# leggedrobotics/art_planner

Measured on NVIDIA H100. Metric: pose-validity checks/s, higher is better.
Workload: dtype f32

## Files before the change

### art_planner_b200/csrc/artp_capi.cu

```cuda
#include <cassert>
#include <climits>
#include <cmath>
#include <cstdlib>
#include <cstring>
#include <type_traits>
#include <vector>

#include "artp_internal.h"
#include "artp_kernels.cuh"
#include "artp_tiles.cuh"

using namespace artp_api;

namespace {

thread_local std::string g_create_error;

__global__ void reverse_columns_kernel(const float* __restrict__ layer, float* __restrict__ H, int nx, int nz, int pitch) {
  const size_t total = (size_t)pitch * nz;
  for (size_t i = blockIdx.x * (size_t)blockDim.x + threadIdx.x; i < total; i += (size_t)gridDim.x * blockDim.x) {
    const int z = (int)(i / pitch), x = (int)(i - (size_t)z * pitch);
    H[i] = (x < nx) ? layer[x + (size_t)(nz - 1 - z) * nx] * 1.0f + 0.0f : 0.0f;
  }
}
// ... 62 lines not shown
  base = lo <= hi ? lo : 0.0f;
  int e = -126;
  while (e < 127 && artp::code_dec(base, std::ldexp(1.0f, e), artp::kCodeMax) < hi) ++e;
  step = std::ldexp(1.0f, e);
}

struct PlaneSlot { unsigned long long key; uint32_t lo, hi; };
constexpr unsigned long long kEmptyKey = ~0ull;
__device__ __forceinline__ unsigned long long plane_key(int kx, int kz, int kd) {
  return ((unsigned long long)(uint32_t)(kx & 0xffff) << 48) | ((unsigned long long)(uint32_t)(kz & 0xffff) << 32) | (uint32_t)kd;
}
__device__ __forceinline__ uint32_t plane_slot_hash(unsigned long long k) {
  k ^= k >> 33; k *= 0xff51afd7ed558ccdull; k ^= k >> 33; k *= 0xc4ceb9fe1a85ec53ull; k ^= k >> 33;
  return (uint32_t)k;
}
__global__ void plane_table_clear_kernel(PlaneSlot* tab, size_t cap) {
  for (size_t i = blockIdx.x * (size_t)blockDim.x + threadIdx.x; i < cap; i += (size_t)gridDim.x * blockDim.x) {
    tab[i].key = kEmptyKey; tab[i].lo = 0xffffffffu; tab[i].hi = 0u;
  }
}
__device__ __forceinline__ bool cell_tri_plane(const artp::Field& f, int x, int x_off, int z, int u, float pl[4]) {
  float hA, hB, hC, hD;
  artp::load_cell(f, x, z, hA, hB, hC, hD);
  const bool ok = u == 0 ? (artp::finitef(hA) && artp::finitef(hB) && artp::finitef(hC))
                         : (artp::finitef(hD) && artp::finitef(hB) && artp::finitef(hC));
  if (!ok) return false;
  artp::cell_plane(f, u == 0, x + x_off, z, hA, hB, hC, hD, pl);
  return true;
}
__global__ void plane_table_insert_kernel(const artp::Field f, int x_off, PlaneSlot* tab, uint32_t mask) {
  const size_t ncell = (size_t)(f.nx - 1) * (f.nz - 1);
  for (size_t i = blockIdx.x * (size_t)blockDim.x + threadIdx.x; i < 2 * ncell; i += (size_t)gridDim.x * blockDim.x) {
    const size_t c = i >> 1;
    const int u = (int)(i & 1), z = (int)(c / (f.nx - 1)), x = (int)(c - (size_t)z * (f.nx - 1));
    float pl[4];
    if (!cell_tri_plane(f, x, x_off, z, u, pl)) continue;
    const uint32_t id = (uint32_t)(((size_t)z * f.pitch + x) * 2 + u);
    const unsigned long long key = plane_key(artp::nkey(pl[0]), artp::nkey(pl[2]), artp::dkey(pl[3]));
    uint32_t s = plane_slot_hash(key) & mask;
    for (;;) {
      const unsigned long long old = atomicCAS(&tab[s].key, kEmptyKey, key);
      if (old == kEmptyKey || old == key) {
        if (!(tab[s].lo < id && tab[s].hi > id)) { atomicMin(&tab[s].lo, id); atomicMax(&tab[s].hi, id); }
        break;
      }
      s = (s + 1) & mask;
    }
  }
}
__global__ void plane_table_query_kernel(const artp::Field f, int x_off, const PlaneSlot* __restrict__ tab, uint32_t mask,
                                         unsigned char* __restrict__ mergeable) {
  const size_t ncell = (size_t)(f.nx - 1) * (f.nz - 1);
  for (size_t i = blockIdx.x * (size_t)blockDim.x + threadIdx.x; i < 2 * ncell; i += (size_t)gridDim.x * blockDim.x) {
    const size_t c = i >> 1;
    const int u = (int)(i & 1), z = (int)(c / (f.nx - 1)), x = (int)(c - (size_t)z * (f.nx - 1));
    float pl[4];
    if (!cell_tri_plane(f, x, x_off, z, u, pl)) continue;
    const uint32_t id = (uint32_t)(((size_t)z * f.pitch + x) * 2 + u);
    const float e2 = 2.0f * ARTP_EPS;
    const int kx0 = artp::nkey(pl[0] - e2), kx1 = artp::nkey(pl[0] + e2);
    const int kz0 = artp::nkey(pl[2] - e2), kz1 = artp::nkey(pl[2] + e2);
    const int kd0 = artp::dkey(pl[3] - e2), kd1 = artp::dkey(pl[3] + e2);
    bool dup = false;
    for (int kx = kx0; kx <= kx1 && !dup; ++kx)
      for (int kz = kz0; kz <= kz1 && !dup; ++kz)
        for (int kd = kd0; kd <= kd1 && !dup; ++kd) {
          const unsigned long long key = plane_key(kx, kz, kd);
          uint32_t s = plane_slot_hash(key) & mask;
          for (;;) {
            const unsigned long long k = tab[s].key;
            if (k == kEmptyKey) break;
            if (k == key) { dup = tab[s].lo != id || tab[s].hi != id; break; }
            s = (s + 1) & mask;
          }
        }
    if (dup) mergeable[(size_t)z * f.pitch + x] = 2;
  }
}

__global__ void fill_u8_kernel(uint8_t* p, size_t n, uint8_t v) {
  for (size_t i = blockIdx.x * (size_t)blockDim.x + threadIdx.x; i < n; i += (size_t)gridDim.x * blockDim.x) p[i] = v;
}

constexpr int kCompactBlock = 1024;
template <bool BITS>
__device__ __forceinline__ int mask_at(const uint8_t* __restrict__ valid, size_t i) {
  if (BITS) return (int)((reinterpret_cast<const uint32_t*>(valid)[i >> 5] >> (i & 31)) & 1u);
  return valid[i] != 0;
}
template <bool BITS>
__global__ void compact_count_kernel(const uint8_t* __restrict__ valid, size_t n, uint32_t* __restrict__ counts) {
  const size_t i = (size_t)blockIdx.x * kCompactBlock + threadIdx.x;
  const int v = (i < n) && mask_at<BITS>(valid, i);
  const int c = __syncthreads_count(v);
  if (threadIdx.x == 0) counts[blockIdx.x] = (uint32_t)c;
}
__global__ void compact_scan_kernel(uint32_t* counts, size_t nb, uint32_t* total) {
  __shared__ uint32_t carry;
  __shared__ uint32_t wsum[32];
  if (threadIdx.x == 0) carry = 0;
  __syncthreads();
  for (size_t b0 = 0; b0 < nb; b0 += blockDim.x) {
    const size_t i = b0 + threadIdx.x;
    const uint32_t v = i < nb ? counts[i] : 0u;
    uint32_t x = v;
    const int lane = threadIdx.x & 31, wid = threadIdx.x >> 5;
    for (int o = 1; o < 32; o <<= 1) { const uint32_t y = __shfl_up_sync(0xffffffffu, x, o); if (lane >= o) x += y; }
    if (lane == 31) wsum[wid] = x;
    __syncthreads();
    if (wid == 0) {
      uint32_t s = lane < (int)(blockDim.x >> 5) ? wsum[lane] : 0u;
      for (int o = 1; o < 32; o <<= 1) { const uint32_t y = __shfl_up_sync(0xffffffffu, s, o); if (lane >= o) s += y; }
      wsum[lane] = s;
    }
    __syncthreads();
    const uint32_t before = carry + (wid ? wsum[wid - 1] : 0u) + x - v;
    if (i < nb) counts[i] = before;
    __syncthreads();
    if (threadIdx.x == blockDim.x - 1) carry = before + v;
    __syncthreads();
  }
  if (threadIdx.x == 0) *total = carry;
}
template <bool BITS, typename IndexT>
__global__ void compact_scatter_kernel(const uint8_t* __restrict__ valid, size_t n, int64_t base,
                                       const uint32_t* __restrict__ offsets, IndexT* __restrict__ out) {
  __shared__ uint32_t wsum[32];
  const size_t i = (size_t)blockIdx.x * kCompactBlock + threadIdx.x;
  const int v = (i < n) && mask_at<BITS>(valid, i);
  const unsigned bal = __ballot_sync(0xffffffffu, v);
  const int lane = threadIdx.x & 31, wid = threadIdx.x >> 5;
  if (lane == 0) wsum[wid] = __popc(bal);
  __syncthreads();
  if (wid == 0) {
    uint32_t s = wsum[lane];
    for (int o = 1; o < 32; o <<= 1) { const uint32_t y = __shfl_up_sync(0xffffffffu, s, o); if (lane >= o) s += y; }
    wsum[lane] = s;
  }
  __syncthreads();
  if (v) {
    const uint32_t pos = offsets[blockIdx.x] + (wid ? wsum[wid - 1] : 0u) + __popc(bal & ((1u << lane) - 1u));
    out[pos] = (IndexT)(base + (int64_t)i);
  }
}

__global__ void pack_bits_kernel(const uint8_t* __restrict__ valid, size_t n, uint32_t* __restrict__ bits) {
  const size_t words = (n + 31) / 32;
  const size_t warps = ((size_t)gridDim.x * blockDim.x) >> 5, wid = ((size_t)blockIdx.x * blockDim.x + threadIdx.x) >> 5;
  const int lane = threadIdx.x & 31;
  for (size_t w = wid; w < words; w += warps) {
    const size_t i = w * 32 + lane;
    const unsigned bal = __ballot_sync(0xffffffffu, i < n && valid[i] != 0);
    if (lane == 0) bits[w] = bal;
  }
}

constexpr size_t kChunkItems = 1u << 20;

int ensure_queues(Handle* h, size_t n_items) {
  const size_t need = 5 * std::min(n_items, kChunkItems);
  if (h->recs_cap >= need) return ARTP_OK;
  const size_t cap = std::max<size_t>(need, 1u << 16);
  h->recs_cap = 0;
  size_t had[4] = {0, 0, 0, 0};
  int rc;
  TRY(grow(h, h->d_recs, had[0], cap));
  TRY(grow(h, h->d_recs_f, had[1], cap));
  TRY(grow(h, h->d_recs_g, had[2], cap));
  TRY(grow(h, h->d_defer, had[3], cap));
  h->recs_cap = cap;
  return ARTP_OK;
}

struct HostFeed {
  const char* host;
  char* dev;
  size_t bytes_per_item;
  size_t slice_items;
  float schedule[8];
};
constexpr size_t kScheduleItems = 1u << 18;
constexpr int kPipeReachCtasPerSm = 2;

__global__ void close_slice_kernel(const BoxQueues* round, BoxQueues* slices, int i) {
  const BoxQueues prev = i ? slices[i - 1] : BoxQueues{};
  slices[i].group = {round->group.end, prev.group.end};
  slices[i].reach = {round->reach.end, prev.reach.end};
  slices[i].big = {round->big.end, prev.big.end};
}

int launch_classify(Handle* h, artp::Work w, size_t lo, size_t hi, cudaStream_t s) {
  w.item_base = (uint32_t)lo;
  w.n_items = (uint32_t)hi;
  BoxQueues* q = &h->d_ctr->q;
  return launch(h, artp::classify_items_kernel, (unsigned)((hi - lo + artp::kClassifyItems - 1) / artp::kClassifyItems),
                artp::kClassifyItems, 0, s, h->chk, w, h->d_recs, h->d_recs_f, h->group_grid ? h->d_recs_g : nullptr, &q->big.end,
                &q->reach.end, &q->group.end, h->mode == 1);
}

int launch_big_tile(Handle* h, artp::Work w, size_t lo, size_t hi, BoxQueues* q, cudaStream_t s) {
  w.item_base = (uint32_t)lo;
  w.n_items = (uint32_t)hi;
  const int wpc = h->tile_warps[0];
  const unsigned grid = (unsigned)std::min<size_t>((size_t)h->tile_grid[0], (5 * (hi - lo) + wpc - 1) / wpc);
  return launch(h, artp::box_tiles_warp_kernel, grid, wpc * 32, h->tile_smem[0], s, h->chk, h->tile_map[0][0], h->tile_map[0][1],
                h->tile_cfg[0], w, h->d_recs, &q->big.end, &q->big.claim, &h->d_ctr->defer, h->d_defer, 0u, h->mode == 1);
}
int launch_reach_warp(Handle* h, artp::Work w, size_t lo, size_t hi, BoxQueues* q, cudaStream_t s, unsigned reach_cap) {
  if (!h->chk.reach_tw) return ARTP_OK;
  w.item_base = (uint32_t)lo;
  w.n_items = (uint32_t)hi;
  const int wpc = h->tile_warps[1];
  const unsigned grid = (unsigned)std::min<size_t>({(size_t)h->tile_grid[1], (4 * (hi - lo) + wpc - 1) / wpc, reach_cap});
  return launch(h, artp::box_tiles_warp_kernel, grid, wpc * 32, h->tile_smem[1], s, h->chk, h->tile_map[1][1], h->tile_map[1][1],
                h->tile_cfg[1], w, h->d_recs_f, &q->reach.end, &q->reach.claim, &h->d_ctr->defer, h->d_defer, artp::kDeferReachBit,
                h->mode == 1);
}
int launch_reach_groups(Handle* h, artp::Work w, size_t lo, size_t hi, BoxQueues* q, cudaStream_t s, unsigned reach_cap) {
  if (!h->group_grid) return ARTP_OK;
  w.item_base = (uint32_t)lo;
  w.n_items = (uint32_t)hi;
  const unsigned grid = (unsigned)std::min<size_t>({(size_t)h->group_grid, (hi - lo + 7) / 8, reach_cap});
  return launch(h, artp::reach_groups_kernel, grid, artp::kMaxTileWarps * 32, h->group_smem, s, h->chk, h->tile_map[1][1],
                h->tile_cfg[1], w, h->d_recs_g, &q->group.end, &q->group.claim);
}

int launch_grouping(Handle* h, artp::Work w, size_t lo, size_t hi, cudaStream_t s) {
  w.item_base = (uint32_t)lo;
  w.n_items = (uint32_t)hi;
  const unsigned grid = (unsigned)std::min<size_t>((size_t)h->k2_grid, 5 * (hi - lo));
  return launch(h, artp::box_items_block_kernel, grid, artp::kBlockStageThreads, h->k2_smem, s, h->chk, w, h->d_recs, h->d_recs_f,
                &h->d_ctr->defer, h->d_defer, h->k2_tcap, h->d_err);
}

int run_round_device(Handle* h, const artp::Work& w, cudaStream_t s, size_t base, size_t end, bool timed) {
  CU_TRY(h, cudaMemsetAsync(h->d_ctr, 0, sizeof(Counters), s));
  if (timed) CU_TRY(h, cudaEventRecord(h->ev[0], s));
  TRY(launch_classify(h, w, base, end, s));
  if (timed) CU_TRY(h, cudaEventRecord(h->ev[1], s));
  const bool fork = !h->timing && h->chk.reach_tw;
  if (fork) {
    CU_TRY(h, cudaEventRecord(h->slice_ev[0], s));
    CU_TRY(h, cudaStreamWaitEvent(h->box_stream, h->slice_ev[0], 0));
    if (h->group_grid) CU_TRY(h, cudaStreamWaitEvent(h->group_stream, h->slice_ev[0], 0));
  }
  BoxQueues* q = &h->d_ctr->q;
  TRY(launch_big_tile(h, w, base, end, q, s));
  if (timed) CU_TRY(h, cudaEventRecord(h->ev[2], s));
  TRY(launch_reach_warp(h, w, base, end, q, fork ? h->box_stream : s, UINT_MAX));
  if (timed) CU_TRY(h, cudaEventRecord(h->ev[3], s));
  TRY(launch_reach_groups(h, w, base, end, q, fork ? h->group_stream : s, UINT_MAX));
  if (fork) {
    CU_TRY(h, cudaEventRecord(h->box_ev, h->box_stream));
    CU_TRY(h, cudaStreamWaitEvent(s, h->box_ev, 0));
    if (h->group_grid) {
      CU_TRY(h, cudaEventRecord(h->group_ev, h->group_stream));
      CU_TRY(h, cudaStreamWaitEvent(s, h->group_ev, 0));
    }
  }
  if (timed) CU_TRY(h, cudaEventRecord(h->ev[4], s));
  TRY(launch_grouping(h, w, base, end, s));
  if (timed) { CU_TRY(h, cudaEventRecord(h->ev[5], s)); h->ev_valid = true; }
  return ARTP_OK;
}

int run_round_piped(Handle* h, const artp::Work& w, cudaStream_t s, const HostFeed& feed, size_t base, size_t end) {
  size_t cut[kMaxSlices + 1];
  int ncut = 0;
  cut[0] = base;
  if (end - base >= kScheduleItems) {
    double acc = 0.0;
    for (int i = 0; i < 8 && feed.schedule[i] > 0.0f; ++i) {
      acc += feed.schedule[i];
      const size_t c = std::min(end, (base + (size_t)((double)(end - base) * acc) + 127) & ~(size_t)127);
      if (c > cut[ncut]) cut[++ncut] = c;
    }
    if (cut[ncut] != end) cut[++ncut] = end;
  } else {
    for (size_t lo = base; lo < end; lo += feed.slice_items) cut[++ncut] = std::min(end, lo + feed.slice_items);
  }
  assert(ncut <= kMaxSlices);
  CU_TRY(h, cudaMemsetAsync(h->d_ctr, 0, sizeof(Counters), s));
  const unsigned reach_cap = (unsigned)(kPipeReachCtasPerSm * h->sm_count);
  for (int si = 0; si < ncut; ++si) {
    const size_t lo = cut[si], hi = cut[si + 1];
    CU_TRY(h, cudaMemcpyAsync(feed.dev + lo * feed.bytes_per_item, feed.host + lo * feed.bytes_per_item,
                              (hi - lo) * feed.bytes_per_item, cudaMemcpyHostToDevice, h->copy_stream));
    CU_TRY(h, cudaEventRecord(h->copy_ev[si], h->copy_stream));
    CU_TRY(h, cudaStreamWaitEvent(s, h->copy_ev[si], 0));
    TRY(launch_classify(h, w, lo, hi, s));
    TRY(launch(h, close_slice_kernel, 1, 1, 0, s, &h->d_ctr->q, h->d_slices, si));
    CU_TRY(h, cudaEventRecord(h->slice_ev[si], s));
    CU_TRY(h, cudaStreamWaitEvent(h->box_stream, h->slice_ev[si], 0));
    if (h->group_grid) CU_TRY(h, cudaStreamWaitEvent(h->group_stream, h->slice_ev[si], 0));
    TRY(launch_reach_groups(h, w, lo, hi, h->d_slices + si, h->group_stream, reach_cap));
    TRY(launch_reach_warp(h, w, lo, hi, h->d_slices + si, h->box_stream, reach_cap));
    TRY(launch_big_tile(h, w, lo, hi, h->d_slices + si, h->box_stream));
  }
  if (h->group_grid) {
    CU_TRY(h, cudaEventRecord(h->group_ev, h->group_stream));
    CU_TRY(h, cudaStreamWaitEvent(h->box_stream, h->group_ev, 0));
  }
  TRY(launch_grouping(h, w, base, end, h->box_stream));
  CU_TRY(h, cudaEventRecord(h->box_ev, h->box_stream));
  CU_TRY(h, cudaStreamWaitEvent(s, h->box_ev, 0));
  return ARTP_OK;
}

int run_items(Handle* h, artp::Work w, cudaStream_t s, const HostFeed* feed = nullptr) {
  const size_t n_total = w.n_items;
  TRY(ensure_queues(h, n_total));
  for (size_t base = 0; base < n_total; base += kChunkItems) {
    const size_t end = std::min(n_total, base + kChunkItems);
    if (feed && feed->slice_items < end - base && !h->timing) {
      TRY(run_round_piped(h, w, s, *feed, base, end));
    } else {
      if (feed)
        CU_TRY(h, cudaMemcpyAsync(feed->dev + base * feed->bytes_per_item, feed->host + base * feed->bytes_per_item,
                                  (end - base) * feed->bytes_per_item, cudaMemcpyHostToDevice, s));
      TRY(run_round_device(h, w, s, base, end, h->timing && end == n_total));
    }
  }
  h->deferred_unread = true;
  return ARTP_OK;
}

int check_common(Handle* h, size_t n) {
  TRY(require_map(h));
  if (n >= (size_t)0xFFFFFFF0u) { h->err = "too many items for one call"; return ARTP_E_LIMIT; }
  return ARTP_OK;
}

int check_poses_small(Handle* h, const artp::SmallBatch& sb, size_t n, uint8_t* valid, int steps = -1) {
  TRY(host_call_begin(h));
  if (!h->h_small_out) {
    CU_TRY(h, cudaHostAlloc((void**)&h->h_small_out, 64, cudaHostAllocMapped));
    CU_TRY(h, cudaFuncSetAttribute(artp::pose_small_kernel, cudaFuncAttributeMaxDynamicSharedMemorySize, 200 * 1024));
  }
  uint8_t* d_out = nullptr;
  CU_TRY(h, cudaHostGetDevicePointer((void**)&d_out, h->h_small_out, 0));
  TRY(launch(h, artp::pose_small_kernel, (unsigned)n, 256, h->k2_smem, h->stream, h->chk, sb, d_out, h->k2_tcap, h->d_err,
      h->mode == 1, steps));
  const int rc = host_call_end(h, true);
  if (rc == ARTP_E_CUDA) return rc;
  if (steps < 0) {
// ... 76 lines not shown
                       size_t total_items, uint8_t* d_item_valid, int32_t* d_valid_prefix, void* stream, int quotient) {
  TRY(check_common(h, total_items));
  if (n == 0) return ARTP_OK;
  if (!d_s1 || !d_s2 || !d_item_off || !d_valid_prefix || (total_items && !d_item_valid)) {
    return null_buffer(h);
  }
  if (n >= 0xFFFFFFFFull) { h->err = "too many edges"; return ARTP_E_INVALID; }
  CU_TRY(h, cudaSetDevice(h->device));
  cudaStream_t s = (cudaStream_t)stream;
  ChainScope cs(h, 0, s);
  if (cs.rc) return cs.rc;
  if (total_items) {
    artp::Work w;
    w.s1 = d_s1; w.s2 = d_s2; w.valid = d_item_valid; w.n_items = (uint32_t)total_items;
    w.item_off = d_item_off; w.n_edges = (uint32_t)n; w.quotient = quotient;
    TRY(run_items(h, w, s));
  }
  TRY(launch(h, edge_prefix_kernel, grid_for(h, n, 256, 8), 256, 0, s, d_item_valid, d_item_off, n, d_valid_prefix));
  h->stats.poses_checked += total_items;
  return ARTP_OK;
}

int check_items_prefix_host(Handle* h, const double* s1, const double* s2, const std::vector<uint32_t>& off, int quotient,
                            int32_t* valid_prefix) {
  const size_t n = off.size() - 1, total = off[n], sb = n * 7 * sizeof(double);
  char* r[5];
  TRY(host_call_begin(h, {sb, sb, (n + 1) * sizeof(uint32_t), n * sizeof(int32_t), total}, r));
  CU_TRY(h, cudaMemcpyAsync(r[0], s1, sb, cudaMemcpyHostToDevice, h->stream));
  CU_TRY(h, cudaMemcpyAsync(r[1], s2, sb, cudaMemcpyHostToDevice, h->stream));
  CU_TRY(h, cudaMemcpyAsync(r[2], off.data(), (n + 1) * sizeof(uint32_t), cudaMemcpyHostToDevice, h->stream));
  TRY(check_items_prefix(h, (const double*)r[0], (const double*)r[1], n, (const uint32_t*)r[2], total, (uint8_t*)r[4],
                         (int32_t*)r[3], h->stream, quotient));
  CU_TRY(h, cudaMemcpyAsync(valid_prefix, r[3], n * sizeof(int32_t), cudaMemcpyDeviceToHost, h->stream));
  return host_call_end(h, true);
}

int pack_valid_bits(Handle* h, const uint8_t* d_valid, size_t n, uint32_t* d_bits, cudaStream_t s) {
  if (n == 0) return ARTP_OK;
  if (!d_valid || !d_bits) return null_buffer(h);
  CU_TRY(h, cudaSetDevice(h->device));
  const size_t words = (n + 31) / 32;
  return launch(h, pack_bits_kernel, grid_for(h, words * 32, 256, 8), 256, 0, s, d_valid, n, d_bits);
}

}

int artp_api::take_sticky_error(Handle* h) {
  if (h->h_err && *(volatile uint32_t*)h->h_err) {
    const uint32_t e = *(volatile uint32_t*)h->h_err;
    *(volatile uint32_t*)h->h_err = 0;
    if (e & 2u) {
      h->err = "a box reached outside this handle's map window (artp_set_map_window: route samples to the shard that holds them, "
               "halo >= box half-diagonal + offsets); affected poses were marked invalid";
      return ARTP_E_WINDOW;
    }
    h->err = "plane-grouping stage overflow: a zone exceeded its shared-memory store; affected poses were marked invalid";
    return ARTP_E_LIMIT;
  }
  return ARTP_OK;
}

int artp_api::check_states_f32(Handle* h, const float* d_states, size_t n, uint8_t* d_valid, cudaStream_t s) {
  return check_states(h, d_states, n, d_valid, s);
}

int artp_api::check_states_cta(Handle* h, const double* d_states, const uint32_t* d_count, const uint32_t* d_stop, size_t max_n,
                               uint8_t* d_valid, cudaStream_t s) {
  if (max_n == 0) return ARTP_OK;
  if (!h->pose_states_smem) {
    CU_TRY(h, cudaFuncSetAttribute(artp::pose_states_kernel, cudaFuncAttributeMaxDynamicSharedMemorySize, 200 * 1024));
    h->pose_states_smem = true;
  }
  TRY(launch(h, artp::pose_states_kernel, (unsigned)max_n, 256, h->k2_smem, s, h->chk, d_states, d_count, d_stop, d_valid,
             h->k2_tcap, h->d_err));
  h->ev_valid = false;
  return ARTP_OK;
}

int artp_api::compact_valid(Handle* h, const uint8_t* d_valid, size_t n, int64_t base, void* d_indices, uint32_t* d_count,
                            cudaStream_t s, bool bits, bool u32) {
  if (n == 0) { CU_TRY(h, cudaMemsetAsync(d_count, 0, sizeof(uint32_t), s)); return ARTP_OK; }
  ChainScope cs(h, 1, s);
  if (cs.rc) return cs.rc;
  const size_t nb = (n + kCompactBlock - 1) / kCompactBlock;
  TRY(grow(h, h->d_block_counts, h->block_counts_cap, nb));
  TRY(bits ? launch(h, compact_count_kernel<true>, (unsigned)nb, kCompactBlock, 0, s, d_valid, n, h->d_block_counts)
           : launch(h, compact_count_kernel<false>, (unsigned)nb, kCompactBlock, 0, s, d_valid, n, h->d_block_counts));
  TRY(launch(h, compact_scan_kernel, 1, 1024, 0, s, h->d_block_counts, nb, d_count));
  if (bits)
    return launch(h, compact_scatter_kernel<true, int64_t>, (unsigned)nb, kCompactBlock, 0, s, d_valid, n, base, h->d_block_counts,
                  (int64_t*)d_indices);
  if (u32)
    return launch(h, compact_scatter_kernel<false, uint32_t>, (unsigned)nb, kCompactBlock, 0, s, d_valid, n, base,
                  h->d_block_counts, (uint32_t*)d_indices);
  return launch(h, compact_scatter_kernel<false, int64_t>, (unsigned)nb, kCompactBlock, 0, s, d_valid, n, base, h->d_block_counts,
                (int64_t*)d_indices);
}

extern "C" {

const char* artp_version(void) { return "artp 0.1 sm_90a"; }

const char* artp_last_error(const artp_handle* hh) {
  if (!hh) return g_create_error.c_str();
  return reinterpret_cast<const Handle*>(hh)->err.c_str();
}

int artp_create(const artp_params* params, artp_handle** out) {
  if (!params || !out) { g_create_error = "null argument"; return ARTP_E_INVALID; }
  *out = nullptr;
  int ndev = 0;
  cudaError_t e = cudaGetDeviceCount(&ndev);
  if (e != cudaSuccess || ndev == 0) {
    g_create_error = std::string("no CUDA device: ") + cudaGetErrorString(e);
    return ARTP_E_CUDA;
  }
  if (params->device < 0 || params->device >= ndev) { g_create_error = "bad device ordinal"; return ARTP_E_INVALID; }
  if (!(params->torso_length > 0 && params->torso_width > 0 && params->torso_height > 0 && params->reach_x > 0 &&
        params->reach_y > 0 && params->reach_z > 0)) {
    g_create_error = "box dimensions must be positive";
    return ARTP_E_INVALID;
  }
  Handle* h = new Handle();
  h->p = *params;
  h->device = params->device;
  auto fail = [&](const char* what, cudaError_t ce) {
    g_create_error = std::string(what) + ": " + cudaGetErrorString(ce);
    artp_destroy(reinterpret_cast<artp_handle*>(h));
    return ARTP_E_CUDA;
  };
  if ((e = cudaSetDevice(h->device)) != cudaSuccess) return fail("cudaSetDevice", e);
  cudaDeviceProp prop;
  if ((e = cudaGetDeviceProperties(&prop, h->device)) != cudaSuccess) return fail("cudaGetDeviceProperties", e);
  h->sm_count = prop.multiProcessorCount;
  cudaFuncAttributes fa;
  if ((e = cudaFuncGetAttributes(&fa, artp::box_tiles_warp_kernel)) != cudaSuccess)
    return fail("no usable kernel image (built for sm_90a)", e);
  for (cudaStream_t* st : {&h->stream, &h->copy_stream, &h->box_stream, &h->group_stream})
    if ((e = cudaStreamCreateWithFlags(st, cudaStreamNonBlocking)) != cudaSuccess) return fail("cudaStreamCreate", e);
  if ((e = cudaEventCreateWithFlags(&h->group_ev, cudaEventDisableTiming)) != cudaSuccess) return fail("cudaEventCreate", e);
  for (int i = 0; i < kMaxSlices; ++i) {
    if ((e = cudaEventCreateWithFlags(&h->copy_ev[i], cudaEventDisableTiming)) != cudaSuccess) return fail("cudaEventCreate", e);
    if ((e = cudaEventCreateWithFlags(&h->slice_ev[i], cudaEventDisableTiming)) != cudaSuccess) return fail("cudaEventCreate", e);
  }
  if ((e = cudaEventCreateWithFlags(&h->box_ev, cudaEventDisableTiming)) != cudaSuccess) return fail("cudaEventCreate", e);
  if ((e = cudaMalloc(&h->d_slices, kMaxSlices * sizeof(BoxQueues))) != cudaSuccess) return fail("cudaMalloc", e);
  if ((e = cudaMalloc(&h->d_ctr, sizeof(Counters))) != cudaSuccess) return fail("cudaMalloc", e);
  for (int g = 0; g < 2; ++g)
    if ((e = cudaEventCreateWithFlags(&h->chain_ev[g], cudaEventDisableTiming)) != cudaSuccess) return fail("cudaEventCreate", e);
  if ((e = cudaHostAlloc((void**)&h->h_err, 64, cudaHostAllocMapped)) != cudaSuccess) return fail("cudaHostAlloc", e);
  *h->h_err = 0;
  if ((e = cudaHostGetDevicePointer((void**)&h->d_err, h->h_err, 0)) != cudaSuccess) return fail("cudaHostGetDevicePointer", e);
  h->cnn = artp_cnn::create(h->device, h->sm_count);
  artp::Checker& c = h->chk;
  std::memset(&c, 0, sizeof(c));
  c.side[0][0] = (float)params->torso_length; c.side[0][1] = (float)params->torso_width; c.side[0][2] = (float)params->torso_height;
  c.side[1][0] = (float)params->reach_x; c.side[1][1] = (float)params->reach_y; c.side[1][2] = (float)params->reach_z;
  c.torso_off[0] = (float)params->torso_off_x; c.torso_off[1] = (float)params->torso_off_y;
  c.torso_off[2] = (float)(params->torso_off_z - params->feet_off_z);
  c.feet_ox = (float)params->feet_off_x; c.feet_oy = (float)params->feet_off_y;
  c.unknown_untraversable = params->unknown_space_untraversable ? 1 : 0;
  *out = reinterpret_cast<artp_handle*>(h);
  return ARTP_OK;
}

void artp_destroy(artp_handle* hh) {
  if (!hh) return;
  Handle* h = reinterpret_cast<Handle*>(hh);
  cudaSetDevice(h->device);
  if (h->stream) { cudaStreamSynchronize(h->stream); cudaStreamDestroy(h->stream); }
  if (h->copy_stream) { cudaStreamSynchronize(h->copy_stream); cudaStreamDestroy(h->copy_stream); }
  if (h->box_stream) { cudaStreamSynchronize(h->box_stream); cudaStreamDestroy(h->box_stream); }
  if (h->group_stream) { cudaStreamSynchronize(h->group_stream); cudaStreamDestroy(h->group_stream); }
  if (h->group_ev) cudaEventDestroy(h->group_ev);
  for (int i = 0; i < kMaxSlices; ++i) {
    if (h->copy_ev[i]) cudaEventDestroy(h->copy_ev[i]);
    if (h->slice_ev[i]) cudaEventDestroy(h->slice_ev[i]);
  }
  if (h->box_ev) cudaEventDestroy(h->box_ev);
  cudaFree(h->d_slices);
  for (int k = 0; k < 2; ++k) for (int l = 0; l <= artp::kMaxLevel; ++l) { cudaFree(h->d_T[k][l]); cudaFree(h->d_C[k][l]); }
  cudaFree(h->d_H[0]); cudaFree(h->d_H[1]); cudaFree(h->d_ctr); cudaFree(h->d_defer); cudaFree(h->d_stage);
  cudaFree(h->d_block_counts); cudaFree(h->d_recs); cudaFree(h->d_recs_f); cudaFree(h->d_recs_g); cudaFree(h->d_samp_layers); cudaFree(h->d_samp_scratch);
  cudaFree(h->d_dist_layers); cudaFree(h->d_dist_scratch); cudaFree(h->d_basic_keep);
  roadmap_free(h);
  if (h->h_small_out) cudaFreeHost(h->h_small_out);
  if (h->h_err) cudaFreeHost(h->h_err);
  for (int g = 0; g < 2; ++g) if (h->chain_ev[g]) cudaEventDestroy(h->chain_ev[g]);
  artp_cnn::destroy(h->cnn);
  for (int i = 0; i < 6; ++i) if (h->ev[i]) cudaEventDestroy(h->ev[i]);
  delete h;
}

int artp_has_map(const artp_handle* hh) {
  if (!hh) return 0;
  Handle* h = reinterpret_cast<Handle*>(const_cast<artp_handle*>(hh));
  std::lock_guard<std::mutex> lock(h->mtx);
  return h->has_map ? 1 : 0;
}

int artp_set_mode(artp_handle* hh, int mode) {
  LOCK_HANDLE(h, hh);
  if (mode < 0 || mode > 1) return ARTP_E_INVALID;
  h->mode = mode;
  return ARTP_OK;
}

int artp_set_timing(artp_handle* hh, int enable) {
  LOCK_HANDLE(h, hh);
  CU_TRY(h, cudaSetDevice(h->device));
  if (enable && !h->ev[0]) for (int i = 0; i < 6; ++i) CU_TRY(h, cudaEventCreate(&h->ev[i]));
  h->timing = enable ? 1 : 0;
  h->ev_valid = false;
  return ARTP_OK;
}

int artp_get_last_timing(artp_handle* hh, float* ms3) {
  LOCK_HANDLE(h, hh);
  if (!ms3) return ARTP_E_INVALID;
  if (!h->timing || !h->ev_valid) { h->err = "timing not enabled or no call recorded"; return ARTP_E_INVALID; }
  CU_TRY(h, cudaSetDevice(h->device));
  CU_TRY(h, cudaEventSynchronize(h->ev[5]));
  CU_TRY(h, cudaEventElapsedTime(ms3 + 0, h->ev[0], h->ev[1]));
  CU_TRY(h, cudaEventElapsedTime(ms3 + 1, h->ev[1], h->ev[4]));
  CU_TRY(h, cudaEventElapsedTime(ms3 + 2, h->ev[4], h->ev[5]));
  return ARTP_OK;
}

int artp_get_last_stage_timing(artp_handle* hh, float* ms5) {
  LOCK_HANDLE(h, hh);
  if (!ms5) return ARTP_E_INVALID;
  if (!h->timing || !h->ev_valid) { h->err = "timing not enabled or no call recorded"; return ARTP_E_INVALID; }
  CU_TRY(h, cudaSetDevice(h->device));
  CU_TRY(h, cudaEventSynchronize(h->ev[5]));
  for (int i = 0; i < 5; ++i) CU_TRY(h, cudaEventElapsedTime(ms5 + i, h->ev[i], h->ev[i + 1]));
  return ARTP_OK;
}

void* artp_host_alloc(size_t bytes) {
  void* p = nullptr;
  if (bytes == 0 || cudaHostAlloc(&p, bytes, cudaHostAllocPortable) != cudaSuccess) return nullptr;
  return p;
}
void artp_host_free(void* p) { if (p) cudaFreeHost(p); }

int artp_poll_error(artp_handle* hh) {
  LOCK_HANDLE(h, hh);
  return take_sticky_error(h);
}

int artp_debug_set_group_capacity(artp_handle* hh, int max_triangles) {
  LOCK_HANDLE(h, hh);
  if (max_triangles < 0) return ARTP_E_INVALID;
  h->tcap_override = max_triangles;
  return ARTP_OK;
}

int artp_get_stats(artp_handle* hh, artp_stats* out) {
  LOCK_HANDLE(h, hh);
  if (!out) return ARTP_E_INVALID;
  CU_TRY(h, cudaSetDevice(h->device));
  Counters ctr{};
  CU_TRY(h, cudaMemcpy(&ctr, h->d_ctr, sizeof(ctr), cudaMemcpyDeviceToHost));
  h->stats.last_deferred = ctr.defer;
  h->stats.last_queued_boxes = ctr.q.big.end + ctr.q.reach.end + ctr.q.group.end;
  h->stats.last_queued_warp_stage = ctr.q.big.end;
// ... 358 lines not shown
```

### art_planner_b200/csrc/artp_internal.h

```cpp
#pragma once

#include <cuda.h>
#include <cuda_runtime.h>

#include <algorithm>
#include <cstdint>
#include <initializer_list>
#include <mutex>
#include <string>
#include <utility>

#include "../../include/artp.h"
#include "artp_cnn.h"
#include "artp_device.cuh"

namespace artp { struct BoxRec; }

namespace artp_api {

constexpr int kMaxSlices = 9;

struct QueueCtr { uint32_t end, claim; };
struct alignas(32) BoxQueues { QueueCtr big, reach, group; };
struct Counters { BoxQueues q; uint32_t defer, scratch; };

struct Roadmap;

struct MapState {
  bool has_sampler = false;
  bool has_device_normals = false;
  bool has_device_cdf = false;
  bool has_normals = false;
  bool has_sample_filter = false;
  bool has_dist_observed = false;
};

struct Handle {
  artp_params p;
  int device = 0;
  int sm_count = 0;
  artp::Checker chk;
  float* d_H[2] = {nullptr, nullptr};
  float2* d_T[2][artp::kMaxLevel + 1] = {};
  uint32_t* d_C[2][artp::kMaxLevel + 1] = {};
  int pitch = 0;
  int rows = 0, cols = 0;
  int win_row0 = 0, win_rows = 0;
  bool has_map = false;
  MapState map;
  Counters* d_ctr = nullptr;
  uint32_t* d_defer = nullptr;
  artp::BoxRec* d_recs = nullptr;
  artp::BoxRec* d_recs_f = nullptr;
  artp::BoxRec* d_recs_g = nullptr;
  int group_grid = 0, group_smem = 0;
  size_t recs_cap = 0;
  uint32_t* d_block_counts = nullptr;
  size_t block_counts_cap = 0;
  char* d_stage = nullptr;
  size_t stage_cap = 0;
  cudaStream_t stream = nullptr;
  cudaStream_t copy_stream = nullptr;
  cudaStream_t group_stream = nullptr;
  cudaEvent_t group_ev = nullptr;
  cudaStream_t box_stream = nullptr;
  cudaEvent_t copy_ev[kMaxSlices] = {};
  cudaEvent_t slice_ev[kMaxSlices] = {};
  cudaEvent_t box_ev = nullptr;
  BoxQueues* d_slices = nullptr;
  int k2_grid = 0, k2_smem = 0, k2_tcap = 0;
  artp::TileCfg tile_cfg[2] = {};
  int tile_grid[2] = {0, 0}, tile_smem[2] = {0, 0}, tile_warps[2] = {8, 8};
  CUtensorMap tile_map[2][2];
  int mode = 0;
  artp_cnn::State* cnn = nullptr;
  int cnn_mode = 0;
  artp::SamplerDev samp{};
  float* d_samp_layers = nullptr;
  size_t samp_layers_cap = 0;
  char* d_samp_scratch = nullptr;
  size_t samp_scratch_cap = 0;
  double res = 0.0;
  float* d_dist_layers = nullptr;
  size_t dist_layers_cap = 0;
  char* d_dist_scratch = nullptr;
  size_t dist_scratch_cap = 0;
  float* d_basic_keep = nullptr;
  size_t basic_keep_cap = 0;
  int basic_rows = 0, basic_cols = 0;
  bool has_basic_layers = false, has_basic_observed = false;
  Roadmap* roadmap = nullptr;
  bool pose_states_smem = false;
  uint8_t* h_small_out = nullptr;
  int timing = 0;
  cudaEvent_t ev[6] = {nullptr, nullptr, nullptr, nullptr, nullptr, nullptr};
  bool ev_valid = false;
  bool deferred_unread = false;
  cudaEvent_t chain_ev[2] = {nullptr, nullptr};
  cudaStream_t chain_stream[2] = {nullptr, nullptr};
  bool chain_busy[2] = {false, false};
  uint32_t* h_err = nullptr;
  uint32_t* d_err = nullptr;
  int tcap_override = 0;
  artp_stats stats{};
  std::string err;
  std::mutex mtx;
};

#define CU_TRY(h, expr)                                                                          \
  do {                                                                                           \
    cudaError_t _e = (expr);                                                                     \
    if (_e != cudaSuccess) {                                                                     \
      (h)->err = std::string(#expr) + ": " + cudaGetErrorString(_e);                             \
      return ARTP_E_CUDA;                                                                        \
    }                                                                                            \
  } while (0)

#define TRY(expr)                                                                                \
  do {                                                                                           \
    if (const int _rc = (expr)) return _rc;                                                      \
  } while (0)

#define LOCK_HANDLE(h, hh)                                                                       \
  if (!(hh)) return ARTP_E_INVALID;                                                              \
  Handle* h = reinterpret_cast<Handle*>(hh);                                                     \
  std::lock_guard<std::mutex> h##_lock(h->mtx)

struct CallScope {
  Handle* h;
  uint64_t launches0;
  explicit CallScope(Handle* h_) : h(h_), launches0(h_->stats.kernel_launches) {}
  ~CallScope() { h->stats.last_launches = (uint32_t)(h->stats.kernel_launches - launches0); }
};
#define LOCK_CALL(h, hh)                                                                         \
  LOCK_HANDLE(h, hh);                                                                            \
  CallScope h##_call(h)

inline int count_launch(Handle* h) {
  CU_TRY(h, cudaGetLastError());
  h->stats.kernel_launches += 1;
  return ARTP_OK;
}

template <typename... P, typename... A>
int launch(Handle* h, void (*kernel)(P...), dim3 grid, dim3 block, size_t smem, cudaStream_t s, A&&... args) {
  kernel<<<grid, block, smem, s>>>(std::forward<A>(args)...);
  return count_launch(h);
// ... 95 lines not shown
```

Baseline: 1.851 billion.

## Single-pass decoupled-lookback compaction and fork big-tile onto high-priority stream

Replaces the three-kernel stream compaction (count, single-block scan, scatter) with one decoupled-lookback kernel. It uses a dynamic tile counter, epoch-tagged per-tile state and 16 ballots per warp, so the serial scan launch and an extra pass over the mask are removed. The big-tile stage moves to a new high-priority stream so it can overlap with the reach kernels, and the wait on the group stream moves after the grouping kernel so grouping no longer waits on it. The lookback adds spin-waiting on tile predecessors and an epoch and reset scheme that depends on tiles being handed out in order. A profiling script is also added.

```diff
diff --git a/art_planner_b200/csrc/artp_capi.cu b/art_planner_b200/csrc/artp_capi.cu
--- a/art_planner_b200/csrc/artp_capi.cu
+++ b/art_planner_b200/csrc/artp_capi.cu
@@ -168,65 +168,92 @@
   for (size_t i = blockIdx.x * (size_t)blockDim.x + threadIdx.x; i < n; i += (size_t)gridDim.x * blockDim.x) p[i] = v;
 }
 
-constexpr int kCompactBlock = 1024;
-template <bool BITS>
-__device__ __forceinline__ int mask_at(const uint8_t* __restrict__ valid, size_t i) {
-  if (BITS) return (int)((reinterpret_cast<const uint32_t*>(valid)[i >> 5] >> (i & 31)) & 1u);
-  return valid[i] != 0;
-}
-template <bool BITS>
-__global__ void compact_count_kernel(const uint8_t* __restrict__ valid, size_t n, uint32_t* __restrict__ counts) {
-  const size_t i = (size_t)blockIdx.x * kCompactBlock + threadIdx.x;
-  const int v = (i < n) && mask_at<BITS>(valid, i);
-  const int c = __syncthreads_count(v);
-  if (threadIdx.x == 0) counts[blockIdx.x] = (uint32_t)c;
-}
-__global__ void compact_scan_kernel(uint32_t* counts, size_t nb, uint32_t* total) {
-  __shared__ uint32_t carry;
-  __shared__ uint32_t wsum[32];
-  if (threadIdx.x == 0) carry = 0;
+constexpr int kCompactThreads = 256, kCompactRounds = 16;
+constexpr int kCompactTile = kCompactThreads * kCompactRounds;
+constexpr unsigned long long kTileAggregate = 1ull << 32, kTileInclusive = 2ull << 32, kTileFlags = 3ull << 32;
+constexpr uint32_t kCompactEpochs = 1u << 30;
+template <bool BITS, typename IndexT>
+__global__ void __launch_bounds__(kCompactThreads)
+compact_kernel(const uint8_t* __restrict__ valid, size_t n, int64_t base, unsigned long long* __restrict__ state, uint32_t epoch,
+               IndexT* __restrict__ out, uint32_t* __restrict__ count) {
+  __shared__ uint32_t s_tile, s_before;
+  __shared__ uint32_t wsum[kCompactThreads / 32];
+  const int lane = threadIdx.x & 31, wid = threadIdx.x >> 5;
+  const size_t ntiles = (n + kCompactTile - 1) / kCompactTile;
+  if (threadIdx.x == 0) {
+    s_tile = (uint32_t)atomicAdd(state, 1ull);
+    if (s_tile == ntiles - 1) *state = 0ull;
+  }
   __syncthreads();
-  for (size_t b0 = 0; b0 < nb; b0 += blockDim.x) {
-    const size_t i = b0 + threadIdx.x;
-    const uint32_t v = i < nb ? counts[i] : 0u;
-    uint32_t x = v;
-    const int lane = threadIdx.x & 31, wid = threadIdx.x >> 5;
+  const uint32_t tile = s_tile;
+  const size_t run0 = (size_t)tile * kCompactTile + (size_t)wid * 32 * kCompactRounds;
+  uint32_t bal[kCompactRounds];
+  if (BITS) {
+    const uint32_t* words = reinterpret_cast<const uint32_t*>(valid);
+    const size_t wi = (run0 >> 5) + lane;
+    uint32_t mine = 0;
+    if (lane < kCompactRounds && wi < (n + 31) / 32) {
+      mine = words[wi];
+      if (n - 32 * wi < 32) mine &= (1u << (n - 32 * wi)) - 1u;
+    }
+#pragma unroll
+    for (int r = 0; r < kCompactRounds; ++r) bal[r] = __shfl_sync(0xffffffffu, mine, r);
+  } else {
+    uint8_t v[kCompactRounds];
+#pragma unroll
+    for (int r = 0; r < kCompactRounds; ++r) {
+      const size_t i = run0 + 32 * r + lane;
+      v[r] = i < n ? valid[i] : 0;
+    }
+#pragma unroll
+    for (int r = 0; r < kCompactRounds; ++r) bal[r] = __ballot_sync(0xffffffffu, v[r] != 0);
+  }
+  uint32_t wtot = 0;
+#pragma unroll
+  for (int r = 0; r < kCompactRounds; ++r) wtot += __popc(bal[r]);
+  if (lane == 0) wsum[wid] = wtot;
+  __syncthreads();
+  const unsigned long long tag = (unsigned long long)epoch << 34;
+  volatile unsigned long long* st = state + 1;
+  if (wid == 0) {
+    uint32_t x = lane < kCompactThreads / 32 ? wsum[lane] : 0u;
+#pragma unroll
     for (int o = 1; o < 32; o <<= 1) { const uint32_t y = __shfl_up_sync(0xffffffffu, x, o); if (lane >= o) x += y; }
-    if (lane == 31) wsum[wid] = x;
-    __syncthreads();
-    if (wid == 0) {
-      uint32_t s = lane < (int)(blockDim.x >> 5) ? wsum[lane] : 0u;
-      for (int o = 1; o < 32; o <<= 1) { const uint32_t y = __shfl_up_sync(0xffffffffu, s, o); if (lane >= o) s += y; }
-      wsum[lane] = s;
-    }
-    __syncthreads();
-    const uint32_t before = carry + (wid ? wsum[wid - 1] : 0u) + x - v;
-    if (i < nb) counts[i] = before;
-    __syncthreads();
-    if (threadIdx.x == blockDim.x - 1) carry = before + v;
-    __syncthreads();
-  }
-  if (threadIdx.x == 0) *total = carry;
-}
-template <bool BITS, typename IndexT>
-__global__ void compact_scatter_kernel(const uint8_t* __restrict__ valid, size_t n, int64_t base,
-                                       const uint32_t* __restrict__ offsets, IndexT* __restrict__ out) {
-  __shared__ uint32_t wsum[32];
-  const size_t i = (size_t)blockIdx.x * kCompactBlock + threadIdx.x;
-  const int v = (i < n) && mask_at<BITS>(valid, i);
-  const unsigned bal = __ballot_sync(0xffffffffu, v);
-  const int lane = threadIdx.x & 31, wid = threadIdx.x >> 5;
-  if (lane == 0) wsum[wid] = __popc(bal);
+    if (lane < kCompactThreads / 32) wsum[lane] = x;
+    const uint32_t agg = __shfl_sync(0xffffffffu, x, kCompactThreads / 32 - 1);
+    uint32_t before = 0;
+    if (tile == 0) {
+      if (lane == 0) st[0] = tag | kTileInclusive | agg;
+    } else {
+      if (lane == 0) st[tile] = tag | kTileAggregate | agg;
+      for (long long j = (long long)tile - 1;; j -= 32) {
+        const long long t = j - lane;
+        unsigned long long s;
+        do {
+          s = t >= 0 ? st[t] : (tag | kTileInclusive);
+        } while (__any_sync(0xffffffffu, (s >> 34) != epoch || !(s & kTileFlags)));
+        const unsigned inc = __ballot_sync(0xffffffffu, (s & kTileFlags) == kTileInclusive);
+        const int stop = inc ? __ffs(inc) - 1 : 31;
+        uint32_t v = lane <= stop ? (uint32_t)s : 0u;
+#pragma unroll
+        for (int o = 16; o; o >>= 1) v += __shfl_xor_sync(0xffffffffu, v, o);
+        before += v;
+        if (inc) break;
+      }
+      if (lane == 0) st[tile] = tag | kTileInclusive | (uint32_t)(before + agg);
+    }
+    if (lane == 0) {
+      s_before = before;
+      if (tile == ntiles - 1) *count = before + agg;
+    }
+  }
   __syncthreads();
-  if (wid == 0) {
-    uint32_t s = wsum[lane];
-    for (int o = 1; o < 32; o <<= 1) { const uint32_t y = __shfl_up_sync(0xffffffffu, s, o); if (lane >= o) s += y; }
-    wsum[lane] = s;
-  }
-  __syncthreads();
-  if (v) {
-    const uint32_t pos = offsets[blockIdx.x] + (wid ? wsum[wid - 1] : 0u) + __popc(bal & ((1u << lane) - 1u));
-    out[pos] = (IndexT)(base + (int64_t)i);
+  uint32_t pos = s_before + (wid ? wsum[wid - 1] : 0u);
+  const unsigned lt = (1u << lane) - 1u;
+#pragma unroll
+  for (int r = 0; r < kCompactRounds; ++r) {
+    if ((bal[r] >> lane) & 1u) out[pos + __popc(bal[r] & lt)] = (IndexT)(base + (int64_t)(run0 + 32 * r + lane));
+    pos += __popc(bal[r]);
   }
 }
 
@@ -327,26 +354,29 @@
   const bool fork = !h->timing && h->chk.reach_tw;
   if (fork) {
     CU_TRY(h, cudaEventRecord(h->slice_ev[0], s));
+    CU_TRY(h, cudaStreamWaitEvent(h->tile_stream, h->slice_ev[0], 0));
     CU_TRY(h, cudaStreamWaitEvent(h->box_stream, h->slice_ev[0], 0));
     if (h->group_grid) CU_TRY(h, cudaStreamWaitEvent(h->group_stream, h->slice_ev[0], 0));
   }
   BoxQueues* q = &h->d_ctr->q;
-  TRY(launch_big_tile(h, w, base, end, q, s));
+  TRY(launch_big_tile(h, w, base, end, q, fork ? h->tile_stream : s));
   if (timed) CU_TRY(h, cudaEventRecord(h->ev[2], s));
   TRY(launch_reach_warp(h, w, base, end, q, fork ? h->box_stream : s, UINT_MAX));
   if (timed) CU_TRY(h, cudaEventRecord(h->ev[3], s));
   TRY(launch_reach_groups(h, w, base, end, q, fork ? h->group_stream : s, UINT_MAX));
   if (fork) {
+    CU_TRY(h, cudaEventRecord(h->tile_ev, h->tile_stream));
+    CU_TRY(h, cudaStreamWaitEvent(s, h->tile_ev, 0));
     CU_TRY(h, cudaEventRecord(h->box_ev, h->box_stream));
     CU_TRY(h, cudaStreamWaitEvent(s, h->box_ev, 0));
-    if (h->group_grid) {
-      CU_TRY(h, cudaEventRecord(h->group_ev, h->group_stream));
-      CU_TRY(h, cudaStreamWaitEvent(s, h->group_ev, 0));
-    }
   }
   if (timed) CU_TRY(h, cudaEventRecord(h->ev[4], s));
   TRY(launch_grouping(h, w, base, end, s));
   if (timed) { CU_TRY(h, cudaEventRecord(h->ev[5], s)); h->ev_valid = true; }
+  if (fork && h->group_grid) {
+    CU_TRY(h, cudaEventRecord(h->group_ev, h->group_stream));
+    CU_TRY(h, cudaStreamWaitEvent(s, h->group_ev, 0));
+  }
   return ARTP_OK;
 }
 
@@ -589,19 +619,22 @@
   if (n == 0) { CU_TRY(h, cudaMemsetAsync(d_count, 0, sizeof(uint32_t), s)); return ARTP_OK; }
   ChainScope cs(h, 1, s);
   if (cs.rc) return cs.rc;
-  const size_t nb = (n + kCompactBlock - 1) / kCompactBlock;
-  TRY(grow(h, h->d_block_counts, h->block_counts_cap, nb));
-  TRY(bits ? launch(h, compact_count_kernel<true>, (unsigned)nb, kCompactBlock, 0, s, d_valid, n, h->d_block_counts)
-           : launch(h, compact_count_kernel<false>, (unsigned)nb, kCompactBlock, 0, s, d_valid, n, h->d_block_counts));
-  TRY(launch(h, compact_scan_kernel, 1, 1024, 0, s, h->d_block_counts, nb, d_count));
+  const size_t nt = (n + kCompactTile - 1) / kCompactTile;
+  if (h->compact_state_cap < nt + 1 || h->compact_epoch + 1 >= kCompactEpochs) {
+    TRY(grow(h, h->d_compact_state, h->compact_state_cap, nt + 1));
+    CU_TRY(h, cudaMemsetAsync(h->d_compact_state, 0, h->compact_state_cap * sizeof(unsigned long long), s));
+    h->compact_epoch = 0;
+  }
+  const uint32_t epoch = ++h->compact_epoch;
+  unsigned long long* st = h->d_compact_state;
   if (bits)
-    return launch(h, compact_scatter_kernel<true, int64_t>, (unsigned)nb, kCompactBlock, 0, s, d_valid, n, base, h->d_block_counts,
-                  (int64_t*)d_indices);
+    return launch(h, compact_kernel<true, int64_t>, (unsigned)nt, kCompactThreads, 0, s, d_valid, n, base, st, epoch,
+                  (int64_t*)d_indices, d_count);
   if (u32)
-    return launch(h, compact_scatter_kernel<false, uint32_t>, (unsigned)nb, kCompactBlock, 0, s, d_valid, n, base,
-                  h->d_block_counts, (uint32_t*)d_indices);
-  return launch(h, compact_scatter_kernel<false, int64_t>, (unsigned)nb, kCompactBlock, 0, s, d_valid, n, base, h->d_block_counts,
-                (int64_t*)d_indices);
+    return launch(h, compact_kernel<false, uint32_t>, (unsigned)nt, kCompactThreads, 0, s, d_valid, n, base, st, epoch,
+                  (uint32_t*)d_indices, d_count);
+  return launch(h, compact_kernel<false, int64_t>, (unsigned)nt, kCompactThreads, 0, s, d_valid, n, base, st, epoch,
+                (int64_t*)d_indices, d_count);
 }
 
 extern "C" {
@@ -645,7 +678,12 @@
     return fail("no usable kernel image (built for sm_90a)", e);
   for (cudaStream_t* st : {&h->stream, &h->copy_stream, &h->box_stream, &h->group_stream})
     if ((e = cudaStreamCreateWithFlags(st, cudaStreamNonBlocking)) != cudaSuccess) return fail("cudaStreamCreate", e);
+  int prio_least = 0, prio_greatest = 0;
+  if ((e = cudaDeviceGetStreamPriorityRange(&prio_least, &prio_greatest)) != cudaSuccess) return fail("cudaDeviceGetStreamPriorityRange", e);
+  if ((e = cudaStreamCreateWithPriority(&h->tile_stream, cudaStreamNonBlocking, prio_greatest)) != cudaSuccess)
+    return fail("cudaStreamCreateWithPriority", e);
   if ((e = cudaEventCreateWithFlags(&h->group_ev, cudaEventDisableTiming)) != cudaSuccess) return fail("cudaEventCreate", e);
+  if ((e = cudaEventCreateWithFlags(&h->tile_ev, cudaEventDisableTiming)) != cudaSuccess) return fail("cudaEventCreate", e);
   for (int i = 0; i < kMaxSlices; ++i) {
     if ((e = cudaEventCreateWithFlags(&h->copy_ev[i], cudaEventDisableTiming)) != cudaSuccess) return fail("cudaEventCreate", e);
     if ((e = cudaEventCreateWithFlags(&h->slice_ev[i], cudaEventDisableTiming)) != cudaSuccess) return fail("cudaEventCreate", e);
@@ -679,7 +717,9 @@
   if (h->copy_stream) { cudaStreamSynchronize(h->copy_stream); cudaStreamDestroy(h->copy_stream); }
   if (h->box_stream) { cudaStreamSynchronize(h->box_stream); cudaStreamDestroy(h->box_stream); }
   if (h->group_stream) { cudaStreamSynchronize(h->group_stream); cudaStreamDestroy(h->group_stream); }
+  if (h->tile_stream) { cudaStreamSynchronize(h->tile_stream); cudaStreamDestroy(h->tile_stream); }
   if (h->group_ev) cudaEventDestroy(h->group_ev);
+  if (h->tile_ev) cudaEventDestroy(h->tile_ev);
   for (int i = 0; i < kMaxSlices; ++i) {
     if (h->copy_ev[i]) cudaEventDestroy(h->copy_ev[i]);
     if (h->slice_ev[i]) cudaEventDestroy(h->slice_ev[i]);
@@ -688,7 +728,7 @@
   cudaFree(h->d_slices);
   for (int k = 0; k < 2; ++k) for (int l = 0; l <= artp::kMaxLevel; ++l) { cudaFree(h->d_T[k][l]); cudaFree(h->d_C[k][l]); }
   cudaFree(h->d_H[0]); cudaFree(h->d_H[1]); cudaFree(h->d_ctr); cudaFree(h->d_defer); cudaFree(h->d_stage);
-  cudaFree(h->d_block_counts); cudaFree(h->d_recs); cudaFree(h->d_recs_f); cudaFree(h->d_recs_g); cudaFree(h->d_samp_layers); cudaFree(h->d_samp_scratch);
+  cudaFree(h->d_compact_state); cudaFree(h->d_recs); cudaFree(h->d_recs_f); cudaFree(h->d_recs_g); cudaFree(h->d_samp_layers); cudaFree(h->d_samp_scratch);
   cudaFree(h->d_dist_layers); cudaFree(h->d_dist_scratch); cudaFree(h->d_basic_keep);
   roadmap_free(h);
   if (h->h_small_out) cudaFreeHost(h->h_small_out);
diff --git a/art_planner_b200/csrc/artp_internal.h b/art_planner_b200/csrc/artp_internal.h
--- a/art_planner_b200/csrc/artp_internal.h
+++ b/art_planner_b200/csrc/artp_internal.h
@@ -55,14 +55,17 @@
   artp::BoxRec* d_recs_g = nullptr;
   int group_grid = 0, group_smem = 0;
   size_t recs_cap = 0;
-  uint32_t* d_block_counts = nullptr;
-  size_t block_counts_cap = 0;
+  unsigned long long* d_compact_state = nullptr;
+  size_t compact_state_cap = 0;
+  uint32_t compact_epoch = 0;
   char* d_stage = nullptr;
   size_t stage_cap = 0;
   cudaStream_t stream = nullptr;
   cudaStream_t copy_stream = nullptr;
   cudaStream_t group_stream = nullptr;
   cudaEvent_t group_ev = nullptr;
+  cudaStream_t tile_stream = nullptr;
+  cudaEvent_t tile_ev = nullptr;
   cudaStream_t box_stream = nullptr;
   cudaEvent_t copy_ev[kMaxSlices] = {};
   cudaEvent_t slice_ev[kMaxSlices] = {};
diff --git a/profiles/step_trace.py b/profiles/step_trace.py
--- /dev/null
+++ b/profiles/step_trace.py
@@ -0,0 +1,124 @@
+import argparse
+import json
+import os
+import re
+import subprocess
+import sys
+import tempfile
+
+ROOT = os.path.dirname(os.path.dirname(os.path.abspath(__file__)))
+sys.path.insert(0, ROOT)
+
+import numpy as np
+import torch
+
+import art_planner_b200 as ap
+from art_planner_b200 import synth
+import bench
+
+KERNELS = ["classify_items_kernel", "box_tiles_warp_kernel", "reach_groups_kernel", "box_items_block_kernel",
+           "pack_bits_kernel", "compact_"]
+
+
+def card():
+    q = subprocess.run(["nvidia-smi", "--query-gpu=name,power.limit", "--format=csv,noheader", "-i",
+                        str(torch.cuda.current_device())], capture_output=True, text=True)
+    name, _, power = q.stdout.strip().partition(",")
+    return {"name": name.strip(), "power_limit": power.strip()}
+
+
+def label(ev, big_corr):
+    n = ev["name"]
+    for k in KERNELS:
+        if k in n:
+            if k == "box_tiles_warp_kernel":
+                return "box_tiles_warp_kernel[big]" if ev["args"].get("correlation") in big_corr else "box_tiles_warp_kernel[reach]"
+            if k == "compact_":
+                return re.search(r"compact_\w+", n).group(0)
+            return k
+    return None
+
+
+def main():
+    ap_ = argparse.ArgumentParser()
+    ap_.add_argument("--steps", type=int, default=50)
+    ap_.add_argument("--warmup", type=int, default=10)
+    ap_.add_argument("--out", default=None, help="directory for step_trace.json and the raw chrome trace")
+    args = ap_.parse_args()
+    assert torch.cuda.is_available(), "step_trace.py needs a CUDA device"
+
+    n = bench.POSES_PER_GPU
+    m, poses = bench.make_inputs(0, n)
+    chk = ap.StateValidityChecker(synth.PARAMS_YAML, device=0)
+    chk.setMap(m)
+    chk.updateHeightField()
+    chk.setTiming(False)
+    d_poses = torch.from_numpy(poses).cuda()
+    d_valid = torch.empty(n, dtype=torch.uint8, device="cuda")
+    bits = torch.empty(n // 32, dtype=torch.int32, device="cuda")
+    idx = torch.empty(n, dtype=torch.int32, device="cuda")
+    cnt = torch.zeros(1, dtype=torch.int32, device="cuda")
+    flush = torch.empty(256 * 1024 * 1024, dtype=torch.uint8, device="cuda")
+
+    def step():
+        chk.isValidBatchBits(d_poses, d_valid, bits)
+        chk.compactValidU32(d_valid, base=0, out_idx=idx, out_cnt=cnt)
+
+    for i in range(args.warmup):
+        flush.fill_(i % 255 + 1)
+        step()
+    torch.cuda.synchronize()
+    acts = [torch.profiler.ProfilerActivity.CUDA]
+    with torch.profiler.profile(activities=acts) as prof:
+        for i in range(args.steps):
+            flush.fill_(i % 255 + 1)
+            step()
+        torch.cuda.synchronize()
+    out_dir = args.out or tempfile.mkdtemp()
+    os.makedirs(out_dir, exist_ok=True)
+    raw = os.path.join(out_dir, "step_trace.pt.trace.json")
+    prof.export_chrome_trace(raw)
+    with open(raw) as f:
+        evs = [e for e in json.load(f)["traceEvents"] if e.get("ph") == "X" and e.get("cat") in ("kernel", "gpu_memset")]
+    evs.sort(key=lambda e: e["ts"])
+    cls = [e for e in evs if "classify_items_kernel" in e["name"]]
+    assert len(cls) == args.steps, f"{len(cls)} classify launches for {args.steps} steps"
+    tiles = [e for e in evs if "box_tiles_warp_kernel" in e["name"]]
+    cs = set()
+    for i, c in enumerate(cls):
+        nxt = cls[i + 1]["ts"] if i + 1 < len(cls) else float("inf")
+        cs.add(min(e["args"]["correlation"] for e in tiles if c["ts"] <= e["ts"] < nxt))
+    rows = {}
+    spans = []
+    for i, c in enumerate(cls):
+        t_end_cls = c["ts"] + c["dur"]
+        nxt = cls[i + 1]["ts"] if i + 1 < len(cls) else float("inf")
+        mset = [e for e in evs if e["cat"] == "gpu_memset" and e["ts"] < c["ts"]]
+        step_evs = [e for e in evs if e["cat"] == "kernel" and c["ts"] <= e["ts"] < nxt and label(e, cs)]
+        started = []
+        for e in step_evs:
+            k = label(e, cs)
+            s0, s1 = e["ts"] - t_end_cls, e["ts"] + e["dur"] - t_end_cls
+            gap = e["ts"] - max((p["ts"] + p["dur"] for p in started), default=e["ts"])
+            started.append(e)
+            rows.setdefault(k, []).append((s0, s1, e["dur"], gap if k != "classify_items_kernel" else 0.0, e["args"].get("grid")))
+        t0 = mset[-1]["ts"] if mset else c["ts"]
+        spans.append(max(e["ts"] + e["dur"] for e in step_evs) - t0)
+    kern = {}
+    for k, v in rows.items():
+        a = np.array([r[:4] for r in v], dtype=np.float64)
+        med = np.median(a, axis=0)
+        kern[k] = {"launches_per_step": len(v) / len(cls), "start_us": round(float(med[0]), 2), "end_us": round(float(med[1]), 2),
+                   "dur_us": round(float(med[2]), 2), "gap_before_us": round(float(med[3]), 2), "grid": v[-1][4]}
+    res = {"card": card(), "steps": len(cls), "times": "median us relative to the end of classify_items_kernel",
+           "step_span_us": round(float(np.median(spans)), 2), "kernels": kern,
+           "last_deferred": chk.stats()["last_deferred"]}
+    line = json.dumps(res)
+    print(line)
+    if args.out:
+        with open(os.path.join(args.out, "step_trace.json"), "w") as f:
+            f.write(line + "\n")
+
+
+if __name__ == "__main__":
+    main()
```

After: 1.908 billion, median of 6. 1.03x the previous value.
